# disanda/Deep-GAN-Encoders

Measured on AMD Instinct MI355X. Metric: encoder-train images/sec (E_align_s2 step, StyleGAN2 FFHQ-1024), higher is better.
Workload: dtype bf16; 1 GPU; E_align_s2 two-phase step, StyleGAN2-1024 G (train mode) + BE(startf=16, L=9) + LPIPS-VGG16 (seeded stand-in weights), batch 8/GPU; global_batch=8, img_size=1024, parallelism=dp1

## Files before the change

### deep-gan-encoders_amd/_lib.py

```python
import ctypes as C
import os

_HERE = os.path.dirname(os.path.abspath(__file__))
LIB_PATH = os.environ.get("DGE_LIB_PATH", os.path.join(_HERE, "libdge_hip.so"))


class DgeError(RuntimeError):
    pass


class ConvDesc(C.Structure):
    _fields_ = [
        ("x", C.c_void_p), ("w_packed", C.c_void_p), ("y", C.c_void_p), ("addend", C.c_void_p), ("dot_src", C.c_void_p),
        ("in_scale", C.c_void_p), ("in_shift", C.c_void_p), ("out_scale", C.c_void_p),
        ("bias", C.c_void_p), ("noise", C.c_void_p), ("noise_w", C.c_void_p), ("stats", C.c_void_p),
        ("B", C.c_int), ("H", C.c_int), ("W", C.c_int), ("Cin", C.c_int), ("Cout", C.c_int),
        ("ksize", C.c_int), ("up", C.c_int), ("in_s2d", C.c_int), ("noise_batch", C.c_int), ("noise_w_per_channel", C.c_int),
        ("act", C.c_int), ("bias_scale", C.c_float), ("gain", C.c_float), ("add_scale", C.c_float),
        ("dtype", C.c_int), ("in_up2", C.c_int), ("in_relu", C.c_int), ("stats_slots", C.c_int), ("w_layout", C.c_int),
        ("prep", C.c_int), ("prep_gain", C.c_float), ("prep_noise", C.c_void_p), ("prep_ns", C.c_void_p), ("prep_noise_batch", C.c_int),
        ("prep_stats", C.c_void_p), ("mask_relu", C.c_int), ("in_t2d", C.c_int),
        ("rgb_w", C.c_void_p), ("rgb_style", C.c_void_p), ("rgb_bias", C.c_void_p), ("rgb_out", C.c_void_p), ("rgb_wscale", C.c_float),
        ("rgb_skip_y", C.c_int), ("pool_out", C.c_int), ("pool_mask", C.c_void_p),
        ("prefetch_w", C.c_void_p), ("prefetch_ntot", C.c_int), ("prefetch_cin", C.c_int), ("in_bwd_coef", C.c_void_p),
# ... 88 lines not shown
    "dge_heads_rows_fwd": [_P, _I, _P, _P, C.c_long, C.c_long, _I, _I, _I, _P],
    "dge_heads_rows_bwd": [_P, _I, _I, _P, C.c_long, C.c_long, _I, _P, _P, _P, _P, _I, _I, _P],
    "dge_dense_wgrad": [_P, _I, _P, _I, _P, _P, _I, _I, _I, _I, _P],
    "dge_lpips_prep": [_P, _P, _I, _I, _I, _P, _P, _I, _P],
    "dge_lpips_prep_bwd": [_P, _P, _I, _I, _I, _P, _F, _I, _I, _P],
    "dge_maxpool2": [_P, _P, _I, _I, _I, _I, _I, _P],
    "dge_maxpool2_bwd": [_P, _P, _P, _P, _I, _I, _I, _I, _I, _P],
    "dge_lpips_head": [_P, _P, _P, _P, _I, _I, _I, _F, _I, _P],
    "dge_mean": [_P, _P, _I, _P],
    "dge_blur_noise_act": [_P, _P, _P, _P, _P, _P, _I, _I, _I, _I, _I, _I, _I, _I, _P],
    "dge_affine_compose": [_P, _P, _P, _P, _P, _I, _I, _P],
    "dge_lerp_layers": [_P, _P, _I, _P, _P, _I, _I, _I, _P],
    "dge_linear_rows": [_P, _I, _P, _P, _P, _P, _P, _P, _I, _I, _I, _F, _F, _F, _P],
    "dge_demod_rows": [_P, _P, _P, _P, _P, _P, _P, _P, _I, _I, _F, _P],
    "dge_fromrgb_dgrad": [_P, _P, _P, _P, _I, _I, _I, _I, _P],
    "dge_nearest_up2": [_P, _P, _I, _I, _I, _I, _F, _I, _P],
    "dge_sg1_in_bwd_coef": [_P, _P, _P, _P, _P, _P, _I, _I, _I, _P],
    "dge_dot_stats": [_P, _P, _P, _I, _I, _I, _I, _P],
    "dge_nearest_up2_bwd": [_P, _P, _P, _P, _I, _I, _I, _I, _I, _P],
    "dge_pixelnorm_nhwc": [_P, _P, C.c_long, _I, _F, _I, _P],
    "dge_pixelnorm_nhwc_bwd": [_P, _P, _P, C.c_long, _I, _F, _I, _P],
    "dge_affine_relu_bwd": [_P, _P, _P, _P, _P, _P, _I, _I, _I, _I, _P],
    "dge_slice_up_bwd": [_P, _P, _I, _I, _I, _I, _I, _I, _I, _P],
    "dge_softmax_rows": [_P, C.c_long, _I, _I, _P],
    "dge_softmax_rows_bwd": [_P, _P, C.c_long, _I, _I, _P],
    "dge_rgb_tanh_bwd": [_P, _P, _P, _I, _I, _I, _I, _P],
    "dge_sn_group": [_P, _I, _I, _I, _P, _F, _I, _P],
    "dge_sn_entry_size": [],
    "dge_cbn_sn_wgrad_entry_size": [],
    "dge_cbn_sn_wgrad_group": [_P, _I, C.c_longlong, _I, _P, _I, _I, _P, _P],
    "dge_upconv_supported": [_I, _I, _I],
    "dge_pack_upconv_weight": [_P, _P, _I, _I, _F, _I, _P],
    "dge_upconv_fir": [_P, _P, _P, _P, _P, _P, _I, _P, _I, _P, _F, _F, _I, _I, _I, _I, _I, _I, _I, _P],
    "dge_cbn_affine": [_P, _P, _I, _P, _P, _F, _P, _P, _I, _I, _P],
    "dge_slice_up": [_P, _P, _I, _I, _I, _I, _I, _I, _I, _P],
    "dge_attention": [_P, _P, _P, _P, _I, _I, _I, _I, _I, _I, _P],
    "dge_rgb_tanh": [_P, _P, _I, _I, _I, _I, _P],
    "dge_guided_relu_bwd": [_P, _P, _P, C.c_long, _I, _I, _P],
    "dge_maxpool2_relu_bwd": [_P, _P, _P, _I, _I, _I, _I, _I, _I, _P],
    "dge_maxpool2_bwd_relu": [_P, _P, _P, _P, _I, _I, _I, _I, _I, _P],
    "dge_adaptive_pool7": [_P, _P, _I, _I, _I, _I, _I, _P],
    "dge_adaptive_pool7_bwd": [_P, _P, _I, _I, _I, _I, _I, _P],
    "dge_class_target": [_P, _P, _P, _P, _I, _I, _P],
    "dge_gather_row": [_P, _P, _P, _I, _I, _F, _P],
    "dge_class_target_rows": [_P, _P, _P, _P, _I, _I, _P],
    "dge_gather_rows": [_P, _P, _P, _I, _I, _P],
    "dge_campp_map": [_P, _P, _P, _P, _P, _I, _I, _I, _I, _I, _P],
    "dge_cam_resize": [_P, _P, _P, _I, _I, _I, _I, _I, _P],
    "dge_mask2cam_blocks": [_I],
    "dge_mask2cam": [_P, _P, _P, _P, _P, _P, _P, _I, _I, _P],
    "dge_mask2cam_rows": [_P, _P, _P, _P, _P, _P, _I, _I, _P],
    "dge_randn": [_P, _I, _P, _P, _P, _P, C.c_ulonglong, _P, _P],
    "dge_version": [],
    "dge_env_reload": [],
    "dge_blend_pool_mask": [_P, _P, _P, _P, _P, _I, _I, _I, _I, _F, _F, _I, _P],
    "dge_act_bwd_mask": [_P, _P, _P, _P, _P, _I, _I, _I, _I, _I, _F, _F, _I, _P],
    "dge_loss_reduce3": [_P, _P, _P, _I, _I, _I, _I, _P, _I, _P],
    "dge_crop_pool_multi": [_P, _P, _P, _P, _I, _I, _I, _I, _P],
    "dge_space_loss_bwd3": [_P, _P, _P, _P, _P, _I, _I, _I, _P, _P, _P, _P, _I, _P],
    "dge_space_loss_bwd_split": [_P, _P, _P, _P, _P, _I, _I, _I, _P, _P, _P, _P, _I, _P],
    "dge_in_bwd_fromrgb": [_P, _P, _P, _I, _P, _P, _P, _P, _I, _P, _P, _P, _I, _I, _I, _I, _I, _F, _I, _P],
    "dge_in_bwd_fromrgb_img": [_P, _P, _P, _I, _P, _P, _P, _P, _I, _P, _P, _P, _P, _P, _I, _I, _I, _I, _I, _F, _I, _P],
    "dge_affine_bwd_fromrgb_img": [_P, _P, _P, _P, _P, _P, _P, _P, _I, _I, _I, _I, _I, _F, _I, _P],
    "dge_in_bwd_fused": [_P, _P, _P, _I, _P, _P, _P, _P, _I, _P, _P, _P, _P, _I, _I, _I, _I, _I, _F, _I, _I, _P],
    "dge_sum_slots_planar_multi": [C.POINTER(SumPlanarEntry), _I, _P],
    "dge_heads_fwd": [_P, _I, _P, _P, _I, _I, _I, _P],
# ... 56 lines not shown
```

### deep-gan-encoders_amd/autograd_s2.py

```python
import torch

from . import ops, s2_conv
from .stylegan2_generator import _dt
from .weight_cache import version


def _style_tables(mod, B, dt):
    nl = mod.num_layers
    groups = [(getattr(mod, f"layer{i}"), i) for i in range(nl - 1)] + [(getattr(mod, f"output{k}"), 2 * k + 1) for k in range(nl // 2)]
    key = (B, str(dt)) + tuple(version(p) for L, _ in groups for p in (L.style.weight, L.style.bias, L.weight))
    cache = mod.__dict__.setdefault("_style_tab", {})
    hit = cache.get(key[:2])
    if hit is not None and hit[0] == key:
        return hit[1]
    dev = groups[0][0].weight.device
    K = mod.w_space_dim
    Wc = torch.cat([L.style.weight.detach() for L, _ in groups]).contiguous()
    bc = torch.cat([L.style.bias.detach() for L, _ in groups]).contiguous()
    xoff, ybase, ybs, s_off = [], [], [], []
    off = 0
    for L, row in groups:
        C = L.in_c
        s_off.append(B * off)
        xoff += [row * K] * C
# ... 91 lines not shown
        g_x, g_srgb, P = ops.torgb_bwd_prep(g_img, layers[top]["y"], Ot.weight.detach().reshape(3, -1), saved["rgb"][top // 2]["s"], Ot.wscale,
                                            layers[top]["noise"], Lt.noise_strength.detach().reshape(1), Lt.gain)
    else:
        g_x, g_srgb = ops.torgb_bwd(g_img, layers[top]["y"], Ot.weight.detach().reshape(3, -1), saved["rgb"][top // 2]["s"], Ot.wscale)
    blocks = [] if fused else None
    if fused:
        blocks.append(dict(gs=g_srgb, wstyle=Ot.style.weight.detach(), row=top + 1))
    else:
        ops.linear_t(g_srgb, Ot.style.weight.detach(), g_wp[:, top + 1], scale=Ot.style.wscale, accumulate=True)
    if top // 2 > 0:
        g_img = ops.up2_bwd(g_img)
    for i in range(top, -1, -1):
        L = getattr(mod, f"layer{i}")
        rec = layers[i]
        if P is not None:
            g_y, d_in = g_x, rec["d"]
        else:
            R = ops.zeros((B, L.out_c, 3), dev)
            g_y, d_in = ops.modconv_bwd_prep(g_x, rec["y"], rec["d"], rec["noise"], L.gain, R), None
        x_in = saved["const"] if i == 0 else layers[i - 1]["y"]
        addend = None
        if i >= 1 and (i - 1) % 2 == 0:
            kp = (i - 1) // 2
            Op = getattr(mod, f"output{kp}")
            addend, g_srgb = ops.torgb_bwd(g_img, x_in, Op.weight.detach().reshape(3, -1), saved["rgb"][kp]["s"], Op.wscale)
            if fused:
                blocks.append(dict(gs=g_srgb, wstyle=Op.style.weight.detach(), row=i))
            else:
                ops.linear_t(g_srgb, Op.style.weight.detach(), g_wp[:, i], scale=Op.style.wscale, accumulate=True)
            if kp > 0:
                g_img = ops.up2_bwd(g_img)
        st = ops.SlotStats(B, L.in_c, dev) if fused else ops.zeros((B, L.in_c, 2), dev)
        prep, P_next = None, None
        if fused and i >= 1 and s2_conv.dgrad_takes_prep(L):
            Lp = getattr(mod, f"layer{i - 1}")
            P_next = ops.SlotStats(B, L.in_c, dev)
            prep = dict(gain=Lp.gain, noise=layers[i - 1]["noise"], ns=Lp.noise_strength.detach().reshape(1), stats=P_next)
        g_xprev = s2_conv.dgrad(L, g_y, d_in, dt, fused, prep=prep, out_scale=rec["s"], addend=addend, stats=st, dot_src=x_in)
        _, wsq = L._prepared(dt)
        if fused and P is not None:
            blocks.append(dict(P=P, st=st, d=rec["d"], s=rec["s"], bias=L.bias.detach(), wsq=wsq, bscale=L.bscale,
                               wstyle=L.style.weight.detach(), row=i))
            g_x, P = g_xprev, P_next
            continue
        if fused:
            st_t = ops.zeros((B, L.in_c, 2), dev)
            ops.check(ops.lib().dge_sum_slots(ops._p(st.buf), ops._p(st_t), st.nslot, st_t.numel(), 0, ops._stream()), "dge_sum_slots")
            st = st_t
        if P is not None:
            t = ops.demod_bwd_prep(P, rec["d"], L.bias.detach(), L.bscale)
        else:
            t = ops.demod_bwd(R, rec["d"], L.bias.detach(), L.noise_strength.detach().reshape(1), L.bscale)
        gs_view = st.view(B, -1)
        ops.linear_t(t, wsq, gs_view, mul=rec["s"], accumulate=True, incy=2, ldy=2 * L.in_c)
        ops.linear_t(gs_view, L.style.weight.detach(), g_wp[:, i], scale=L.style.wscale, accumulate=True, incx=2,
                     ldx=2 * L.in_c, O=L.in_c)
        g_x, P = g_xprev, P_next
    if blocks:
        ops.s2_style_grads(blocks, g_wp, getattr(mod, "layer0").style.wscale)
    return g_wp


class SynthesisFunction(torch.autograd.Function):
    @staticmethod
    def forward(ctx, mod, wp, randomize_noise):
        need = ctx.needs_input_grad[1]
        results, saved = synthesis_run(mod, wp.detach(), randomize_noise, save=need)
# ... 32 lines not shown
```

### deep-gan-encoders_amd/ops.py

```python
import ctypes as C
import math

import torch

from ._lib import lib, check, ConvDesc, ConvPPDesc, DgeError, last_kernel

F32, BF16 = 0, 1
ACT_NONE, ACT_LRELU, ACT_RELU, LIN_RSQRT = 0, 1, 2, 3
PACK_FWD, PACK_UPFOLD, PACK_DGRAD, PACK_UPFOLD_DGRAD, PACK_SG1_UP, PACK_SG1_UP_DGRAD, PACK_UPT2D_DGRAD = 0, 1, 2, 3, 4, 5, 6
PACK_FRAG = 0x100
import os as _os
import weakref as _weakref
KERNEL_LOG = None
PROFILE = None


class _ZeroArena:

    def __init__(self):
        self.buf, self.off, self.high, self.active = None, 0, 0, False


_ARENA = _ZeroArena()

# ... 1146 lines not shown

def maxpool2_bwd(gy, x, addend=None, relu=False):
    B, H, W, Cc = x.shape
    gx = torch.empty_like(x)
    fn = lib().dge_maxpool2_bwd_relu if relu else lib().dge_maxpool2_bwd
    check(fn(_p(gy), _p(x), _p(addend), _p(gx), B, H, W, Cc, dtype_of(x), _stream()), "dge_maxpool2_bwd")
    return gx


def upconv_supported(cin, cout, dtype):
    return bool(lib().dge_upconv_supported(int(cin), int(cout), int(dtype)))


def pack_upconv_weight(w, dtype=BF16, scale=1.0):
    cout, cin = w.shape[0], w.shape[1]
    out = torch.empty((9, cout, cin), dtype=tdtype(dtype), device=w.device)
    check(lib().dge_pack_upconv_weight(_f32(w.detach().contiguous()), _p(out), cout, cin, float(scale), dtype, _stream()),
          "dge_pack_upconv_weight")
    return out


def upconv_fir(x, w_packed, cout, in_scale=None, out_scale=None, bias=None, bias_scale=1.0, noise=None, noise_w=None,
               act=ACT_NONE, gain=1.0):
    B, H, W, Cin = x.shape
    y = torch.empty((B, 2 * H, 2 * W, cout), dtype=x.dtype, device=x.device)
    nbs = 0 if (noise is None or noise.shape[0] == 1) else 4 * H * W
    nws = 0 if (noise_w is None or noise_w.numel() == 1) else 1
    _launch(lib().dge_upconv_fir, (_p(x), _p(w_packed), _p(y), _f32(in_scale), _f32(out_scale), _f32(noise), nbs, _f32(noise_w), nws,
                                   _f32(bias), float(bias_scale), float(gain), int(act), B, H, W, Cin, cout, dtype_of(x), _stream()),
            "dge_upconv_fir", 9.0 * Cin * cout * H * W * B, (B, H, W, Cin, cout, 3, "upfir", False), (x, y, w_packed))
    return y


TRACK_ARM_AT, TRACK_ARM_AFTER = 0, 1


def latent_pnorm(w, p=2, out=None, out_l2=None):
    if out is None:
        out = torch.empty((), dtype=torch.float32, device=w.device)
    check(lib().dge_latent_pnorm_fwd(_f32(w.contiguous()), _p(out), _f32(out_l2), w.numel(), int(p), _stream()), "dge_latent_pnorm_fwd")
    return out


def latent_l2(w, out=None):
    if out is None:
        out = torch.empty((), dtype=torch.float32, device=w.device)
    check(lib().dge_latent_pnorm_fwd(_f32(w.contiguous()), None, _p(out), w.numel(), 2, _stream()), "dge_latent_pnorm_fwd")
    return out


def latent_pnorm_bwd(w, norm, g, p=2, beta=1.0, gout=None):
    check(lib().dge_latent_pnorm_bwd(_f32(w.contiguous()), _f32(norm), _f32(gout), _f32(g), w.numel(), int(p), float(beta), _stream()),
          "dge_latent_pnorm_bwd")
    return g


def wplus_lerp(w, avg, psi, out=None):
    B, L, D = w.shape
    if out is None:
        out = torch.empty((B, L, D), dtype=torch.float32, device=w.device)
    stride = D if avg.numel() == L * D else 0
    check(lib().dge_wplus_lerp(_f32(w.contiguous()), _f32(avg.contiguous()), stride, float(psi), _p(out), B, L, D, _stream()),
          "dge_wplus_lerp")
    return out


# ... 59 lines not shown
```

### deep-gan-encoders_amd/s2_conv.py

```python
import os

from . import ops
from .weight_cache import lookup, store

PP_GEN = not os.environ.get("DGE_NO_PP_GEN")
UP_PP = os.environ.get("DGE_UP_PP", "1") != "0"
UP_FOLDED = os.environ.get("DGE_UP_FOLDED") == "1"
T2D = not os.environ.get("DGE_NO_T2D")
PP_DG = not os.environ.get("DGE_NO_PP_DG")


def prepared(L, dtype):
    c = lookup(L._cache, ("w", dtype), L.weight)
    if c is None:
        mode = ops.PACK_UPFOLD if L.up else ops.PACK_FWD
        hin = L.res // 2 if L.up else L.res
        packed = ops.pack_conv_weight(L.weight, ops.pack_mode_for(L.weight, mode, hin, hin, dtype), dtype, L.wscale) \
            if L.ksize == 3 else None
        wsq = ops.weight_sumsq(L.weight, L.wscale) if L.demodulate else None
        c = store(L._cache, ("w", dtype), L.weight, (packed, wsq))
    return c


def _prepared_up(L, dtype):
    if not L.up or L.res < 32 or UP_FOLDED or not ops.upconv_supported(L.in_c, L.out_c, dtype):
        return None
    c = lookup(L._cache, ("wu", dtype), L.weight)
    return c if c is not None else store(L._cache, ("wu", dtype), L.weight, ops.pack_upconv_weight(L.weight, dtype, L.wscale))


def forward(L, x, s, d, noise, dt, rgb=None):
    nw = L.noise_strength.detach().reshape(1) if noise is not None else None
    B, H, W, _ = x.shape
    wu = _prepared_up(L, dt)
    if wu is not None:
        assert rgb is None
        if (UP_PP and s is not None and d is not None and (noise is None or nw.numel() == 1)
                and ops.up_pp_supported(B, H, W, L.in_c, L.out_c, dt)):
            wimg = ops.pack_up_pp(wu, L.out_c, L.in_c, in_scale=s, out_scale=d, gain=L.gain)
            return ops.up_pp(x, wimg, L.out_c, bias=L.bias, bias_scale=L.bscale, noise=noise, noise_w=nw, act=L.act, gain=L.gain)
        return ops.upconv_fir(x, wu, L.out_c, in_scale=s, out_scale=d, bias=L.bias, bias_scale=L.bscale, noise=noise, noise_w=nw, act=L.act, gain=L.gain)
    if (rgb is None and not L.up and d is not None and s is not None and L.ksize == 3 and PP_GEN
# ... 4 lines not shown
    return ops.conv2d(x, packed, L.out_c, 3, up=L.up, in_scale=s, out_scale=d, bias=L.bias, bias_scale=L.bscale, noise=noise, noise_w=nw, act=L.act, gain=L.gain, rgb=rgb)


def _up_phase_form(L):
    return L.up and 32 <= L.res // 2 <= 128 and L.in_c >= 64 and L.in_c % 32 == 0 and L.out_c % 8 == 0 and T2D


def _dgrad_weight(L, dtype):
    hg = L.res // 2 if L.up else L.res
    if _up_phase_form(L):
        mode = ops.PACK_UPT2D_DGRAD
    else:
        mode = ops.pack_mode_for(L.weight, ops.PACK_UPFOLD_DGRAD if L.up else ops.PACK_DGRAD, hg, hg, dtype)
    c = lookup(L._cache, ("dg", dtype, mode), L.weight)
    return c if c is not None else store(L._cache, ("dg", dtype, mode), L.weight, ops.pack_conv_weight(L.weight, mode, dtype, L.wscale))


def _pp_dgrad(L, B, hg, dtype):
    K = 4 * L.out_c if L.up else L.out_c
    return PP_DG and (not L.up or L.out_c % 32 == 0) and ops.conv_pp_supported(B, hg, hg, K, L.in_c, dtype)


def _dgrad_weight_pp(L, d, t2d=False):
    if not L.up:
        return ops.pack_conv_pp(L.weight, L.wscale, in_scale=d, dgrad=True)
    name = "dgpp_t2d" if t2d else "dgpp"
    c = lookup(L._cache, name, L.weight)
    if c is None:
        rows = ops.pack_conv_weight(L.weight, ops.PACK_UPT2D_DGRAD if t2d else ops.PACK_UPFOLD_DGRAD, ops.F32, L.wscale)
        c = store(L._cache, name, L.weight, ops.pack_conv_pp_rows(rows, L.in_c, t2d=True) if t2d else rows)
    return c if t2d else ops.pack_conv_pp_rows(c, L.in_c, in_scale=d, in_period=L.out_c)


def dgrad_takes_prep(L):
    return _up_phase_form(L) or not (L.up and L.in_c < 128)


def dgrad(L, g_y, d_in, dt, fused, prep=None, **epilogue):
    B, hg = g_y.shape[0], (L.res // 2 if L.up else L.res)
    t2d = _up_phase_form(L)
    if fused and d_in is not None and not t2d and _pp_dgrad(L, B, hg, dt):
        return ops.conv_pp(g_y, _dgrad_weight_pp(L, d_in), L.in_c, dgrad=True, in_s2d=L.up, add_scale=1.0, prep=prep, **epilogue)
    if t2d and fused and prep is not None and _pp_dgrad(L, B, hg, dt):
        return ops.conv_pp(ops.fir_t2d(g_y, d_in), _dgrad_weight_pp(L, None, t2d=True), L.in_c, dgrad=True, in_t2d=True, add_scale=1.0, prep=prep, **epilogue)
    if t2d:
        return ops.conv2d(ops.fir_t2d(g_y, d_in), _dgrad_weight(L, dt), L.in_c, 3, in_t2d=True, add_scale=1.0, prep=prep, **epilogue)
    return ops.conv2d(g_y, _dgrad_weight(L, dt), L.in_c, 3, in_s2d=L.up, in_scale=d_in, add_scale=1.0, prep=prep, **epilogue)
```

### include/dge_hip.h

```cpp
#ifndef DGE_HIP_H
#define DGE_HIP_H
#include <stddef.h>
#ifdef __cplusplus
extern "C" {
#endif

typedef struct ihipStream_t* dge_stream_t;

#define DGE_DTYPE_F32 0
#define DGE_DTYPE_BF16 1
#define DGE_ACT_LINEAR 0
#define DGE_ACT_LRELU02 1
#define DGE_ACT_RELU_ 2
#define DGE_LIN_RSQRT 3
#define DGE_PACK_FWD 0
#define DGE_PACK_UPFOLD 1
#define DGE_PACK_DGRAD 2
#define DGE_PACK_UPFOLD_DGRAD 3
#define DGE_PACK_SG1_UP 4
#define DGE_PACK_SG1_UP_DGRAD 5
#define DGE_PACK_UPT2D_DGRAD 6

const char* dge_last_error(void);
int dge_version(void);
// ... 212 lines not shown
int dge_maxpool2(const void* x, void* y, int B, int H, int W, int C, int dtype, dge_stream_t stream);
int dge_maxpool2_bwd(const void* gy, const void* x, const void* addend, void* gx, int B, int H, int W, int C, int dtype,
                     dge_stream_t stream);
int dge_lpips_head(const void* feat, const float* lin, float* val, void* g1, int B, int HW, int C, float gscale, int dtype,
                   dge_stream_t stream);
int dge_mean(const float* v, float* out, int n, dge_stream_t stream);

int dge_blur_noise_act(const void* x, const float* noise, const float* noise_w, const float* bias, void* y, float* stats,
                       int B, int H, int W, int C, int do_blur, int noise_batch, int act, int dtype, dge_stream_t stream);
int dge_affine_compose(const float* sc, const float* sh, const float* style, float* a, float* b, int B, int C, dge_stream_t stream);
int dge_lerp_layers(const float* w, const float* avg, int avg_stride, const float* coefs, float* out, int B, int L, int D,
                    dge_stream_t stream);

int dge_sg1_in_bwd_coef(const float* dots, const float* sc, const float* sh, const float* style, float* coef, float* gstyle,
                        int B, int C, int npix, dge_stream_t stream);
int dge_dot_stats(const void* g, const void* x, float* stats, int B, int HW, int C, int dtype, dge_stream_t stream);
int dge_nearest_up2_bwd(const void* ghi, const void* x, void* glow, float* stats, int B, int H, int W, int C, int dtype,
                        dge_stream_t stream);

int dge_sn_group(const void* entries, int n, int maxO, int maxK, float* sigma, float eps, int training, dge_stream_t stream);
int dge_sn_entry_size(void);
int dge_cbn_sn_wgrad_entry_size(void);
int dge_cbn_sn_wgrad_group(const void* entries, int n, long long rows, int maxC, const float* cond, int B, int K, float* rowdot, dge_stream_t stream);

int dge_randn(float* out, int nseg, const long long* start, const long long* count, const unsigned long long* goff,
              const unsigned int* subseq, unsigned long long seed, const unsigned long long* seed_dev, dge_stream_t stream);

int dge_upconv_supported(int Cin, int Cout, int dtype);
int dge_pack_upconv_weight(const float* w, void* out, int Cout, int Cin, float scale, int dtype, dge_stream_t stream);
int dge_upconv_fir(const void* x, const void* w_packed, void* y, const float* in_scale, const float* out_scale,
                   const float* noise, int noise_bstride, const float* noise_w, int noise_w_stride, const float* bias,
                   float bias_scale, float gain, int act, int B, int H, int W, int Cin, int Cout, int dtype, dge_stream_t stream);

int dge_up_pp_supported(int B, int H, int W, int Cin, int Cout, int dtype);
int dge_pack_up_pp(const void* w_units, void* out, int Cout, int Cin, const float* in_scale, const float* out_scale, float gain,
                   int nb, dge_stream_t stream);
int dge_up_pp(const void* x, const void* w_img, long long w_bstride, void* y, const float* noise, int noise_bstride,
              const float* noise_w, const float* bias, float bias_scale, float gain, int act, int B, int H, int W, int Cin, int Cout,
              dge_stream_t stream);

typedef struct dge_conv_pp_desc {
    const void* x;
    const void* w_pp;
    void* y;
    long long w_bstride;
    const float* out_scale;
    const float* bias;
    const float* noise;
    const float* noise_w;
    int B, H, W, Cin, Cout;
    int noise_batch;
    int noise_w_per_channel;
    int act;
    float bias_scale, gain;
    int dgrad, in_s2d, stats_slots, prep, prep_noise_batch, mask_relu;
    int in_t2d;
    float add_scale, prep_gain;
    const void* dot_src;
    const void* addend;
    float* stats;
    float* prep_stats;
    const float* prep_noise;
    const float* prep_ns;
} dge_conv_pp_desc;
int dge_conv_pp_supported(int B, int H, int W, int Cin, int Cout, int dtype);
int dge_pack_conv_pp(const float* w_oihw, void* out, int N, int K, float wscale, const float* in_scale, const float* out_scale,
// ... 67 lines not shown
```

Baseline: 374.9 images/sec.

## Add streaming fused upsample-conv dgrad kernel for 64<-32 channel layers

Adds a dedicated HIP kernel for the backward data gradient of the upsampling 3x3 modulated conv at the highest-resolution 64->32 channel StyleGAN2 layer. It streams gradient rows through LDS with direct-to-LDS buffer loads, applies the transposed FIR blur in registers, runs MFMA, and fuses the epilogue: out_scale, addend, dot-product stats, and the previous layer's prep (lrelu gain, noise, stats). This removes the separate FIR-transpose pass and the generic conv path, plus their intermediate memory traffic. It only handles one channel configuration, is disabled in deterministic mode, and lets that layer take the fused prep path.

```diff
diff --git a/deep-gan-encoders_amd/_lib.py b/deep-gan-encoders_amd/_lib.py
--- a/deep-gan-encoders_amd/_lib.py
+++ b/deep-gan-encoders_amd/_lib.py
@@ -144,6 +144,8 @@
     "dge_upconv_supported": [_I, _I, _I],
     "dge_pack_upconv_weight": [_P, _P, _I, _I, _F, _I, _P],
     "dge_upconv_fir": [_P, _P, _P, _P, _P, _P, _I, _P, _I, _P, _F, _F, _I, _I, _I, _I, _I, _I, _I, _P],
+    "dge_up_dgrad_stream_supported": [_I, _I, _I, _I, _I, _I],
+    "dge_up_dgrad_stream": [_P, _P, _P, _P, _P, _P, _P, _P, _I, _I, _F, _P, _I, _P, _P, _I, _I, _I, _I, _I, _I, _P],
     "dge_cbn_affine": [_P, _P, _I, _P, _P, _F, _P, _P, _I, _I, _P],
     "dge_slice_up": [_P, _P, _I, _I, _I, _I, _I, _I, _I, _P],
     "dge_attention": [_P, _P, _P, _P, _I, _I, _I, _I, _I, _I, _P],
diff --git a/deep-gan-encoders_amd/autograd_s2.py b/deep-gan-encoders_amd/autograd_s2.py
--- a/deep-gan-encoders_amd/autograd_s2.py
+++ b/deep-gan-encoders_amd/autograd_s2.py
@@ -147,7 +147,7 @@
                 g_img = ops.up2_bwd(g_img)
         st = ops.SlotStats(B, L.in_c, dev) if fused else ops.zeros((B, L.in_c, 2), dev)
         prep, P_next = None, None
-        if fused and i >= 1 and s2_conv.dgrad_takes_prep(L):
+        if fused and i >= 1 and s2_conv.dgrad_takes_prep(L, B, dt):
             Lp = getattr(mod, f"layer{i - 1}")
             P_next = ops.SlotStats(B, L.in_c, dev)
             prep = dict(gain=Lp.gain, noise=layers[i - 1]["noise"], ns=Lp.noise_strength.detach().reshape(1), stats=P_next)
diff --git a/deep-gan-encoders_amd/csrc/upconv_stream_bwd.hip b/deep-gan-encoders_amd/csrc/upconv_stream_bwd.hip
--- /dev/null
+++ b/deep-gan-encoders_amd/csrc/upconv_stream_bwd.hip
@@ -0,0 +1,382 @@
+#include <type_traits>
+#include <stdlib.h>
+#include "common.h"
+#include "../../include/dge_hip.h"
+
+namespace {
+
+typedef __attribute__((ext_vector_type(4))) unsigned rsrc_t;
+typedef __attribute__((ext_vector_type(2))) float f2_t;
+
+__device__ __forceinline__ unsigned rfl(unsigned v) { return __builtin_amdgcn_readfirstlane(v); }
+__device__ __forceinline__ unsigned lds_off(const void* p) {
+    return (unsigned)(size_t)(const __attribute__((address_space(3))) unsigned char*)p;
+}
+__device__ __forceinline__ rsrc_t make_rsrc(unsigned long long base, unsigned bytes) {
+    rsrc_t r;
+    r[0] = rfl((unsigned)base); r[1] = rfl((unsigned)(base >> 32) & 0xffffu); r[2] = rfl(bytes); r[3] = 0x00020000u;
+    return r;
+}
+
+struct UpbParams {
+    const void* gz; const void* w; void* y; const void* addend; const void* dot_src;
+    const float* d_in; const float* out_scale;
+    float* stats; float* prep_stats; int stats_slots;
+    const float* prep_noise; const float* prep_ns; int prep_noise_bstride; float prep_gain;
+    int B, H, W;
+    int nstrips, nseg, seg_rows, njobs, jobs_per_xcd;
+    int dbg;
+};
+
+constexpr int CIN = 64, COUT = 32;
+constexpr int ZRB = 34 * 128;
+constexpr int NS = 3, D = 2;
+constexpr int ZPAIR = 2 * ZRB;
+constexpr int Z_OFF = 0;
+constexpr int T_OFF = (NS * ZPAIR + 255) / 256 * 256;
+constexpr int T_ODD = 34 * 64;
+constexpr int TRB = T_ODD + 32 * 64, NT = 4;
+constexpr int D_OFF = T_OFF + NT * TRB;
+constexpr int DROWB = 2048, DRING = NS * DROWB;
+constexpr int A_OFF = D_OFF + 2 * DRING;
+constexpr int N_OFF = A_OFF + 2 * DRING;
+constexpr int NRING = NS * 256;
+constexpr int DUMMY_OFF = (N_OFF + 2 * NRING + 255) / 256 * 256;
+constexpr int LDS_BYTES = DUMMY_OFF + 1024;
+constexpr int LPR = 6 + 2 + 2 + 1;
+static_assert((D - 1) * LPR < 64, "vmcnt range");
+
+__device__ __forceinline__ int swz8(int px) { return (px >> 1) & 7; }
+__device__ __forceinline__ int swz4(int px) { return (px >> 2) & 3; }
+
+#define UPB_P(off) "buffer_load_dwordx4 %1, %3, 0 offen offset:" #off " lds\n\t"
+#define UPB_M0 "s_mov_b32 m0, %2\n\ts_nop 0\n\t"
+__device__ __forceinline__ void dma_row(int wave, unsigned voff, unsigned voff_b, unsigned voff_c, rsrc_t rs, rsrc_t rs_null,
+                                        unsigned m0v, unsigned m0_dummy) {
+    unsigned long long keep;
+    if (wave == 0)
+        asm volatile(UPB_M0 UPB_P(0) UPB_P(2048)
+                     "s_mov_b32 m0, %5\n\ts_mov_b64 %0, exec\n\ts_mov_b64 exec, 0xffff\n\tbuffer_load_dwordx4 %4, %3, 0 offen lds\n\ts_mov_b64 exec, %0"
+                     : "=&s"(keep) : "v"(voff), "s"(m0v), "s"(rs), "v"(voff_c), "s"(m0v + 4096u) : "memory");
+    else
+        asm volatile(UPB_M0 UPB_P(1024) UPB_P(3072) "s_mov_b32 m0, %5\n\ts_nop 0\n\tbuffer_load_dwordx4 %1, %4, 0 offen lds"
+                     : "=&s"(keep) : "v"(voff_b), "s"(m0v), "s"(rs), "s"(rs_null), "s"(m0_dummy) : "memory");
+}
+__device__ __forceinline__ void dma_half(unsigned voff, unsigned voff1, rsrc_t rs, unsigned m0v) {
+    asm volatile("s_mov_b32 m0, %1\n\ts_nop 0\n\tbuffer_load_dwordx4 %0, %2, 0 offen lds\n\t"
+                 "buffer_load_dwordx4 %3, %2, 0 offen offset:1024 lds" : : "v"(voff), "s"(m0v), "s"(rs), "v"(voff1) : "memory");
+}
+__device__ __forceinline__ void dma_f32(unsigned voff, rsrc_t rs, unsigned m0v) {
+    asm volatile("s_mov_b32 m0, %1\n\ts_nop 0\n\tbuffer_load_dword %0, %2, 0 offen lds" : : "v"(voff), "s"(m0v), "s"(rs) : "memory");
+}
+
+__device__ __forceinline__ int chan_of_row(int m) {
+    const int j = m >> 3, k = (m >> 2) & 1, i = m & 3;
+    return 16 * (j >> 1) + 8 * k + 4 * (j & 1) + i;
+}
+__device__ __forceinline__ int chan_of_reg(int kh, int r) { return (r < 8 ? 8 * kh + r : 16 + 8 * kh + (r - 8)); }
+
+template <bool PREP>
+__global__ __launch_bounds__(128, 1) void upconv_stream_bwd_kernel(UpbParams p) {
+    extern __shared__ __attribute__((aligned(1024))) unsigned char lds[];
+    const int lane = threadIdx.x & 63;
+    const int wave = (int)rfl(threadIdx.x >> 6);
+    const unsigned lds0 = lds_off(lds);
+    const int n31 = lane & 31, kh = lane >> 5;
+
+    int job = (blockIdx.x & 7) * p.jobs_per_xcd + (blockIdx.x >> 3);
+    if ((int)(blockIdx.x >> 3) >= p.jobs_per_xcd || job >= p.njobs) return;
+    const int strip = job % p.nstrips; job /= p.nstrips;
+    const int seg = job % p.nseg;
+    const int b = job / p.nseg;
+    const int r0 = seg * p.seg_rows;
+    const int r1 = min(r0 + p.seg_rows, p.H);
+    const int nsteps = r1 - r0 + 2;
+    const int x0 = 32 * strip;
+    const int FH = 2 * p.H;
+
+    const unsigned zrow_bytes = (unsigned)(2 * p.W) * (COUT * 2);
+    const unsigned yrow_bytes = (unsigned)p.W * (CIN * 2);
+    const unsigned long long Zb = (unsigned long long)p.gz + (unsigned long long)b * FH * zrow_bytes;
+    const unsigned long long DOTb = (unsigned long long)p.dot_src + (unsigned long long)b * p.H * yrow_bytes;
+    const unsigned long long ADDb = p.addend ? (unsigned long long)p.addend + (unsigned long long)b * p.H * yrow_bytes : Zb;
+    const bool has_nz = PREP && p.prep_noise != nullptr;
+    const unsigned long long NZb = has_nz ? (unsigned long long)(p.prep_noise + (size_t)b * p.prep_noise_bstride) : Zb;
+    const unsigned nzrow_bytes = (unsigned)p.W * 4;
+
+    unsigned voff, voff_b, voff_c;
+    {
+        const int px = lane >> 3, cs = lane & 7;
+        const int gx = x0 - 1 + px;
+        voff = (unsigned)(gx * 128 + ((cs ^ swz8(px)) << 4));
+        voff_b = (unsigned)(gx * 128 + ((cs ^ swz8(px + 8)) << 4));
+        voff_c = voff + 4096;
+    }
+    unsigned dvoff, dvoff1;
+    {
+        const int px = lane >> 2, cs = lane & 3;
+        dvoff = (unsigned)((x0 + px) * 128 + wave * 64 + ((cs ^ swz4(px)) << 4));
+        dvoff1 = dvoff + 2048u - 1024u;
+    }
+    const unsigned nvoff = lane < 32 ? (unsigned)((x0 + lane) * 4) : 0x80000000u;
+    const rsrc_t rs_null = make_rsrc(Zb, 0);
+
+    auto issue = [&](int tt, int slot) {
+        const int gy = 2 * (r0 - 1 + tt);
+        const bool live = tt < nsteps;
+        const bool zv = live && gy >= 0 && gy < FH;
+        const unsigned long long zp = Zb + (unsigned long long)(zv ? gy : 0) * zrow_bytes;
+        const unsigned m0z = lds0 + Z_OFF + (unsigned)slot * ZPAIR;
+        dma_row(wave, voff, voff_b, voff_c, make_rsrc(zp, zv ? zrow_bytes : 0u), rs_null, m0z, lds0 + DUMMY_OFF);
+        dma_row(wave, voff, voff_b, voff_c, make_rsrc(zp + zrow_bytes, zv ? zrow_bytes : 0u), rs_null, m0z + ZRB, lds0 + DUMMY_OFF);
+        const bool ov = live && tt >= 2;
+        const unsigned long long ro = (unsigned long long)(ov ? r0 - 2 + tt : 0);
+        dma_half(dvoff, dvoff1, make_rsrc(DOTb + ro * yrow_bytes, ov ? yrow_bytes : 0u), lds0 + D_OFF + (unsigned)(wave * DRING + slot * DROWB));
+        dma_half(dvoff, dvoff1, make_rsrc(ADDb + ro * yrow_bytes, (ov && p.addend) ? yrow_bytes : 0u), lds0 + A_OFF + (unsigned)(wave * DRING + slot * DROWB));
+        dma_f32(nvoff, make_rsrc(NZb + ro * nzrow_bytes, (ov && has_nz) ? nzrow_bytes : 0u), lds0 + N_OFF + (unsigned)(wave * NRING + slot * 256));
+    };
+    asm volatile("s_waitcnt vmcnt(0)" ::: "memory");
+    for (int h = 0; h < D; h++) issue(h, h);
+
+    uint4 wf[9][2];
+    {
+        const bf16_t* __restrict__ Wp = (const bf16_t*)p.w;
+        const int ci = wave * 32 + chan_of_row(n31);
+#pragma unroll
+        for (int tap = 0; tap < 9; tap++)
+#pragma unroll
+            for (int ks = 0; ks < 2; ks++) wf[tap][ks] = *(const uint4*)(Wp + ((size_t)(tap * CIN + ci) * COUT + ks * 16 + kh * 8));
+    }
+    float oscv[16];
+#pragma unroll
+    for (int r = 0; r < 16; r++) oscv[r] = p.out_scale ? p.out_scale[b * CIN + wave * 32 + chan_of_reg(kh, r)] : 1.f;
+    const float pg_pos = p.prep_gain, pg_neg = 0.2f * p.prep_gain, pz_pos = 1.f / p.prep_gain, pz_neg = 1.f / (0.2f * p.prep_gain);
+    const float pns = (has_nz && p.prep_ns) ? p.prep_ns[0] : 0.f;
+
+    typedef unsigned u32x4_t __attribute__((ext_vector_type(4)));
+    typedef const __attribute__((address_space(3))) u32x4_t* lds_u4p;
+    typedef __attribute__((address_space(3))) u32x4_t* lds_u4wp;
+    typedef const __attribute__((address_space(3))) float* lds_fp;
+    auto lds_u4 = [&](unsigned a) { const u32x4_t t = *(lds_u4p)(size_t)a; return make_uint4(t[0], t[1], t[2], t[3]); };
+    auto lds_st4 = [&](unsigned a, unsigned v0, unsigned v1, unsigned v2, unsigned v3) { u32x4_t t; t[0] = v0; t[1] = v1; t[2] = v2; t[3] = v3; *(lds_u4wp)(size_t)a = t; };
+
+    const int fc = lane & 3, fj = lane >> 2;
+    unsigned zoff[6];
+#pragma unroll
+    for (int k = 0; k < 6; k++) {
+        const int sp = 16 * wave + fj + (k >> 1);
+        zoff[k] = lds0 + Z_OFF + (unsigned)(sp * 128 + ((((k & 1) * 4 + fc) ^ swz8(sp)) << 4));
+    }
+    const int tj = 16 * wave + fj;
+    const unsigned toff_e = lds0 + T_OFF + (unsigned)(tj * 64 + ((fc ^ swz4(tj)) << 4));
+    const unsigned toff_o = toff_e + T_ODD;
+    const unsigned toff_x = lds0 + T_OFF + (unsigned)((tj + 1) * 64 + ((fc ^ swz4(tj + 1)) << 4));
+    const bool wr_x = tj == 31;
+    f2_t dsc[4];
+#pragma unroll
+    for (int i = 0; i < 4; i++) dsc[i] = p.d_in ? f2_t{p.d_in[b * COUT + 8 * fc + 2 * i], p.d_in[b * COUT + 8 * fc + 2 * i + 1]} : f2_t{1.f, 1.f};
+    f2_t hist[3][3][4];
+#pragma unroll
+    for (int r = 0; r < 3; r++)
+#pragma unroll
+        for (int c = 0; c < 3; c++)
+#pragma unroll
+            for (int i = 0; i < 4; i++) hist[r][c][i] = f2_t{0.f, 0.f};
+
+    unsigned boff[3][2];
+#pragma unroll
+    for (int kx = 0; kx < 3; kx++)
+#pragma unroll
+        for (int ks = 0; ks < 2; ks++) {
+            const int jj = n31 + (kx >> 1);
+            boff[kx][ks] = lds0 + T_OFF + (unsigned)((kx & 1) * T_ODD + jj * 64 + (((2 * ks + kh) ^ swz4(jj)) << 4));
+        }
+    unsigned eoff[2];
+#pragma unroll
+    for (int q = 0; q < 2; q++) eoff[q] = (unsigned)(wave * DRING + n31 * 64 + (((2 * q + kh) ^ swz4(n31)) << 4));
+    const unsigned nzoff = lds0 + N_OFF + (unsigned)(wave * NRING + n31 * 4);
+
+    const bool pv = x0 + n31 < p.W;
+    const bool stv = pv && !(p.dbg & 1);
+    unsigned char* __restrict__ Yb = (unsigned char*)p.y + (size_t)b * p.H * yrow_bytes + (size_t)(x0 + n31) * (CIN * 2) + wave * 64 + kh * 16;
+    float s0[16], s1[16], s2[PREP ? 16 : 1];
+#pragma unroll
+    for (int r = 0; r < 16; r++) { s0[r] = 0.f; s1[r] = 0.f; if (PREP) s2[r] = 0.f; }
+    f32x16_t zero16;
+#pragma unroll
+    for (int r = 0; r < 16; r++) zero16[r] = 0.f;
+
+    int slot = 0, slot_pf = D % NS;
+    for (int t = 0; t < nsteps; t++) {
+        asm volatile("s_waitcnt vmcnt(%0)" :: "i"((D - 1) * LPR) : "memory");
+        __builtin_amdgcn_s_barrier();
+        issue(t + D, slot_pf);
+
+        if (!(p.dbg & 8)) {
+            f2_t hn[2][3][4];
+#pragma unroll
+            for (int r = 0; r < 2; r++) {
+                f2_t g[6][4];
+#pragma unroll
+                for (int k = 0; k < 6; k++) {
+                    const uint4 v = lds_u4(zoff[k] + (unsigned)(slot * ZPAIR + r * ZRB));
+                    const unsigned w4[4] = {v.x, v.y, v.z, v.w};
+#pragma unroll
+                    for (int i = 0; i < 4; i++) g[k][i] = f2_t{__uint_as_float(w4[i] << 16), __uint_as_float(w4[i] & 0xffff0000u)};
+                }
+#pragma unroll
+                for (int c = 0; c < 3; c++)
+#pragma unroll
+                    for (int i = 0; i < 4; i++) hn[r][c][i] = (g[c][i] + g[c + 3][i]) * 0.25f + (g[c + 1][i] + g[c + 2][i]) * 0.75f;
+            }
+            const unsigned ta = (unsigned)(((2 * t + 1) & (NT - 1)) * TRB), tb = (unsigned)(((2 * t + 2) & (NT - 1)) * TRB);
+#pragma unroll
+            for (int c = 0; c < 3; c++) {
+                unsigned oa[4], ob[4];
+#pragma unroll
+                for (int i = 0; i < 4; i++) {
+                    const f2_t va = ((hist[0][c][i] + hn[0][c][i]) * 0.25f + (hist[1][c][i] + hist[2][c][i]) * 0.75f) * dsc[i];
+                    const f2_t vb = ((hist[1][c][i] + hn[1][c][i]) * 0.25f + (hist[2][c][i] + hn[0][c][i]) * 0.75f) * dsc[i];
+                    oa[i] = pack2bf(va[0], va[1]); ob[i] = pack2bf(vb[0], vb[1]);
+                    hist[0][c][i] = hist[2][c][i]; hist[1][c][i] = hn[0][c][i]; hist[2][c][i] = hn[1][c][i];
+                }
+                const unsigned o = c == 0 ? toff_e : (c == 1 ? toff_o : toff_x);
+                if (c < 2 || wr_x) { lds_st4(o + ta, oa[0], oa[1], oa[2], oa[3]); lds_st4(o + tb, ob[0], ob[1], ob[2], ob[3]); }
+            }
+        }
+        asm volatile("s_waitcnt lgkmcnt(0)" ::: "memory");
+        __builtin_amdgcn_s_barrier();
+
+        if (t >= 2) {
+            constexpr int NQ = 18, PF = 6;
+            unsigned rowb[3];
+#pragma unroll
+            for (int ky = 0; ky < 3; ky++) rowb[ky] = (unsigned)(((2 * t + ky) & (NT - 1)) * TRB);
+            f32x16_t acc = zero16;
+            if (!(p.dbg & 2)) {
+                uint4 bq[PF];
+                StaticFor<PF>::run([&](auto qc) { constexpr int q = decltype(qc)::value; bq[q] = lds_u4(boff[(q >> 1) % 3][q & 1] + rowb[(q >> 1) / 3]); });
+                StaticFor<NQ>::run([&](auto qc) {
+                    constexpr int q = decltype(qc)::value;
+                    constexpr int tap = q >> 1, ks = q & 1;
+                    const bf16x8_t bf = *(const bf16x8_t*)&bq[q % PF];
+                    acc = __builtin_amdgcn_mfma_f32_32x32x16_bf16(*(const bf16x8_t*)&wf[tap][ks], bf, acc, 0, 0, 0);
+                    if constexpr (q + PF < NQ) { constexpr int q2 = q + PF; bq[q % PF] = lds_u4(boff[(q2 >> 1) % 3][q2 & 1] + rowb[(q2 >> 1) / 3]); }
+                });
+            }
+            const unsigned so = (unsigned)(slot * DROWB);
+            uint4 dd[2], aa[2];
+#pragma unroll
+            for (int q = 0; q < 2; q++) { dd[q] = lds_u4(lds0 + D_OFF + eoff[q] + so); aa[q] = lds_u4(lds0 + A_OFF + eoff[q] + so); }
+            float nzs = 0.f;
+            if (PREP) nzs = pns * *(lds_fp)(size_t)(nzoff + (unsigned)(slot * 256));
+            float v[16];
+#pragma unroll
+            for (int q = 0; q < 2; q++) {
+                float dv[8], av[8];
+                unpack16(dd[q], dv, (bf16_t*)nullptr);
+                unpack16(aa[q], av, (bf16_t*)nullptr);
+#pragma unroll
+                for (int e = 0; e < 8; e++) {
+                    const int r = 8 * q + e;
+                    const float a = acc[r];
+                    s0[r] = fmaf(a, dv[e], s0[r]);
+                    const float g = fmaf(a, oscv[r], av[e]);
+                    if (PREP) {
+                        const bool pos = dv[e] > 0.f;
+                        const float gz = g * (pos ? pg_pos : pg_neg);
+                        const float zt = dv[e] * (pos ? pz_pos : pz_neg) - nzs;
+                        s2[PREP ? r : 0] = fmaf(gz, zt, s2[PREP ? r : 0]); s1[r] += gz;
+                        v[r] = gz;
+                    } else {
+                        s1[r] += a;
+                        v[r] = g;
+                    }
+                }
+            }
+            if (stv) {
+                unsigned char* dst = Yb + (size_t)(r0 - 2 + t) * yrow_bytes;
+                *(uint4*)dst = make_uint4(pack2bf(v[0], v[1]), pack2bf(v[2], v[3]), pack2bf(v[4], v[5]), pack2bf(v[6], v[7]));
+                *(uint4*)(dst + 32) = make_uint4(pack2bf(v[8], v[9]), pack2bf(v[10], v[11]), pack2bf(v[12], v[13]), pack2bf(v[14], v[15]));
+            }
+        }
+        slot = slot + 1 == NS ? 0 : slot + 1;
+        slot_pf = slot_pf + 1 == NS ? 0 : slot_pf + 1;
+    }
+    asm volatile("s_waitcnt vmcnt(0)" ::: "memory");
+
+    if (p.stats) {
+        float* __restrict__ ST = p.stats + ((size_t)(blockIdx.x % p.stats_slots) * p.B + b) * CIN * 2;
+        float* __restrict__ PST = (PREP && p.prep_stats) ? p.prep_stats + ((size_t)(blockIdx.x % p.stats_slots) * p.B + b) * CIN * 2 : nullptr;
+        float va = 0.f, vc = 0.f, vt = 0.f;
+#pragma unroll
+        for (int r = 0; r < 16; r++) {
+            float a = pv ? s0[r] : 0.f, c = pv ? s1[r] : 0.f, t2 = (PREP && pv) ? s2[PREP ? r : 0] : 0.f;
+#pragma unroll
+            for (int m = 1; m < 32; m <<= 1) {
+                a += __shfl_xor(a, m, 64); c += __shfl_xor(c, m, 64);
+                if (PREP) t2 += __shfl_xor(t2, m, 64);
+            }
+            if (n31 == r) { va = a; vc = c; vt = t2; }
+        }
+        if (n31 < 16) {
+            const int ch = wave * 32 + chan_of_reg(kh, n31);
+            atomicAdd(ST + ch * 2, va);
+            if (PREP) { if (PST) { atomicAdd(PST + ch * 2, vt); atomicAdd(PST + ch * 2 + 1, vc); } }
+            else atomicAdd(ST + ch * 2 + 1, vc);
+        }
+    }
+}
+
+template <bool PREP>
+int launch(UpbParams& p, hipStream_t s) {
+    auto kern = upconv_stream_bwd_kernel<PREP>;
+    static int caps[16] = {0};
+    int dev = 0;
+    (void)hipGetDevice(&dev);
+    int& cap = caps[dev >= 0 && dev < 16 ? dev : 0];
+    if (!cap) {
+        (void)hipFuncSetAttribute((const void*)kern, hipFuncAttributeMaxDynamicSharedMemorySize, LDS_BYTES);
+        int occ = 0, ncu = 256;
+        (void)hipDeviceGetAttribute(&ncu, hipDeviceAttributeMultiprocessorCount, dev);
+        if (hipOccupancyMaxActiveBlocksPerMultiprocessor(&occ, (const void*)kern, 128, LDS_BYTES) != hipSuccess || occ < 1) occ = 1;
+        cap = occ * ncu;
+    }
+    p.nstrips = (p.W + 31) / 32;
+    int nseg = cap / (p.B * p.nstrips);
+    int maxseg = p.H / 16; if (maxseg < 1) maxseg = 1;
+    if (nseg > maxseg) nseg = maxseg;
+    if (nseg < 1) nseg = 1;
+    p.seg_rows = (p.H + nseg - 1) / nseg;
+    p.nseg = (p.H + p.seg_rows - 1) / p.seg_rows;
+    p.njobs = p.B * p.nstrips * p.nseg;
+    p.jobs_per_xcd = (p.njobs + 7) / 8;
+    dge_note_kernel(PREP ? "upconv_stream_bwd<bf16,%d,%d>+prep" : "upconv_stream_bwd<bf16,%d,%d>", CIN, COUT);
+    hipLaunchKernelGGL(kern, dim3((unsigned)(p.jobs_per_xcd * 8)), dim3(128), LDS_BYTES, s, p);
+    DGE_LAUNCH_CHECK("upconv_stream_bwd");
+    return 0;
+}
+
+}
+
+extern "C" int dge_up_dgrad_stream_supported(int B, int H, int W, int Cin, int Cout, int dtype) {
+    if (dtype != DGE_BF16 || Cin != CIN || Cout != COUT || B < 1 || H < 1 || W < 1) return 0;
+    if ((long)W * 128 >= (1L << 31) || (long)B * H * W * 128 >= (1L << 40)) return 0;
+    return 1;
+}
+
+extern "C" int dge_up_dgrad_stream(const void* g_z, const void* w_packed, void* y, const float* d_in, const float* out_scale,
+                                   const void* addend, const void* dot_src, float* stats, int stats_slots, int prep, float prep_gain,
+                                   const float* prep_noise, int prep_noise_bstride, const float* prep_ns, float* prep_stats,
+                                   int B, int H, int W, int Cin, int Cout, int dtype, hipStream_t s) {
+    DGE_CHECK(dge_up_dgrad_stream_supported(B, H, W, Cin, Cout, dtype), "up_dgrad_stream: bf16, %d -> %d channels only (got %d -> %d)", CIN, COUT, Cin, Cout);
+    DGE_CHECK(dot_src && stats && stats_slots >= 1, "up_dgrad_stream: needs dot_src and stats");
+    DGE_CHECK(!prep || (prep_stats && prep_gain > 0.f), "up_dgrad_stream: prep needs its stats and a positive gain");
+    UpbParams p;
+    p.gz = g_z; p.w = w_packed; p.y = y; p.addend = addend; p.dot_src = dot_src; p.d_in = d_in; p.out_scale = out_scale;
+    p.stats = stats; p.prep_stats = prep ? prep_stats : nullptr; p.stats_slots = stats_slots;
+    p.prep_noise = prep ? prep_noise : nullptr; p.prep_ns = prep_ns; p.prep_noise_bstride = prep_noise_bstride; p.prep_gain = prep ? prep_gain : 1.f;
+    p.B = B; p.H = H; p.W = W;
+    p.dbg = dge_env().up_dbg;
+    return prep ? launch<true>(p, s) : launch<false>(p, s);
+}
diff --git a/deep-gan-encoders_amd/ops.py b/deep-gan-encoders_amd/ops.py
--- a/deep-gan-encoders_amd/ops.py
+++ b/deep-gan-encoders_amd/ops.py
@@ -1202,6 +1202,47 @@
     return y
 
 
+def up_dgrad_stream_supported(B, Hin, Win, cin, cout, dtype):
+    return (not is_deterministic()) and bool(lib().dge_up_dgrad_stream_supported(int(B), int(Hin), int(Win), int(cin), int(cout), int(dtype)))
+
+
+def pack_up_dgrad_stream(w, dtype=BF16, scale=1.0):
+    if dtype != BF16:
+        raise DgeError("pack_up_dgrad_stream: bf16 only")
+    cout, cin = w.shape[0], w.shape[1]
+    return (w.detach().float() * float(scale)).flip(2, 3).permute(2, 3, 1, 0).reshape(9, cin, cout).to(torch.bfloat16).contiguous()
+
+
+def up_dgrad_stream(g_z, w_packed, d_in, out_scale, addend, stats, dot_src, prep=None):
+    B, FH, FW, cout = g_z.shape
+    H, W = FH // 2, FW // 2
+    _, cin, _ = w_packed.shape
+    dt = dtype_of(g_z)
+    if dot_src is None or stats is None:
+        raise DgeError("up_dgrad_stream: needs stats and dot_src")
+    if not up_dgrad_stream_supported(B, H, W, cin, cout, dt):
+        raise DgeError(f"up_dgrad_stream: unsupported launch {cin} <- {cout} channels, dtype {dt}")
+    out = torch.empty((B, H, W, cin), dtype=g_z.dtype, device=g_z.device)
+    nslot = _stats_slots(B, H, W, 32)
+    lazy = isinstance(stats, SlotStats)
+    partial = stats.alloc(nslot) if lazy else (zeros((nslot,) + tuple(stats.shape), g_z.device) if nslot > 1 else stats)
+    pn = pns = pst = None
+    pgain, pbs = 1.0, 0
+    if prep is not None:
+        pn = prep.get("noise")
+        pns = prep.get("ns") if pn is not None else None
+        pbs = 0 if (pn is None or pn.shape[0] == 1) else H * W
+        pgain, pst = float(prep["gain"]), prep["stats"].alloc(nslot)
+    _launch(lib().dge_up_dgrad_stream,
+            (_p(g_z), _p(w_packed), _p(out), _f32(d_in), _f32(out_scale), _p(addend), _p(dot_src), _f32(partial), nslot,
+             0 if prep is None else 1, pgain, _f32(pn), pbs, _f32(pns), _f32(pst), B, H, W, cin, cout, dt, _stream()),
+            "dge_up_dgrad_stream", 9.0 * cin * cout * H * W * B, (B, H, W, 4 * cout, cin, 3, False, True),
+            (g_z, out, addend, dot_src, w_packed))
+    if not lazy and partial is not stats:
+        check(lib().dge_sum_slots(_p(partial), _p(stats), nslot, stats.numel(), 1, _stream()), "dge_sum_slots")
+    return out
+
+
 TRACK_ARM_AT, TRACK_ARM_AFTER = 0, 1
 
 
diff --git a/deep-gan-encoders_amd/s2_conv.py b/deep-gan-encoders_amd/s2_conv.py
--- a/deep-gan-encoders_amd/s2_conv.py
+++ b/deep-gan-encoders_amd/s2_conv.py
@@ -8,6 +8,7 @@
 UP_FOLDED = os.environ.get("DGE_UP_FOLDED") == "1"
 T2D = not os.environ.get("DGE_NO_T2D")
 PP_DG = not os.environ.get("DGE_NO_PP_DG")
+UP_DG_STREAM = not os.environ.get("DGE_NO_UP_DG_STREAM")
 
 
 def prepared(L, dtype):
@@ -78,12 +79,27 @@
     return c if t2d else ops.pack_conv_pp_rows(c, L.in_c, in_scale=d, in_period=L.out_c)
 
 
-def dgrad_takes_prep(L):
+def _up_stream_dgrad(L, B, dtype, fused):
+    return UP_DG_STREAM and fused and L.up and L.ksize == 3 and ops.up_dgrad_stream_supported(B, L.res // 2, L.res // 2, L.in_c, L.out_c, dtype)
+
+
+def _dgrad_weight_stream(L, dtype):
+    c = lookup(L._cache, ("dgs", dtype), L.weight)
+    return c if c is not None else store(L._cache, ("dgs", dtype), L.weight, ops.pack_up_dgrad_stream(L.weight, dtype, L.wscale))
+
+
+def dgrad_takes_prep(L, B=None, dtype=None):
+    if B is not None and L.up and _up_stream_dgrad(L, B, dtype, not ops.is_deterministic()):
+        return True
     return _up_phase_form(L) or not (L.up and L.in_c < 128)
 
 
 def dgrad(L, g_y, d_in, dt, fused, prep=None, **epilogue):
     B, hg = g_y.shape[0], (L.res // 2 if L.up else L.res)
+    if L.up and _up_stream_dgrad(L, B, dt, fused) and epilogue.get("dot_src") is not None and epilogue.get("stats") is not None \
+            and set(epilogue) <= {"out_scale", "addend", "stats", "dot_src"}:
+        return ops.up_dgrad_stream(g_y, _dgrad_weight_stream(L, dt), d_in, epilogue.get("out_scale"), epilogue.get("addend"),
+                                   epilogue.get("stats"), epilogue["dot_src"], prep=prep)
     t2d = _up_phase_form(L)
     if fused and d_in is not None and not t2d and _pp_dgrad(L, B, hg, dt):
         return ops.conv_pp(g_y, _dgrad_weight_pp(L, d_in), L.in_c, dgrad=True, in_s2d=L.up, add_scale=1.0, prep=prep, **epilogue)
diff --git a/include/dge_hip.h b/include/dge_hip.h
--- a/include/dge_hip.h
+++ b/include/dge_hip.h
@@ -268,6 +268,12 @@
                    const float* noise, int noise_bstride, const float* noise_w, int noise_w_stride, const float* bias,
                    float bias_scale, float gain, int act, int B, int H, int W, int Cin, int Cout, int dtype, dge_stream_t stream);
 
+int dge_up_dgrad_stream_supported(int B, int H, int W, int Cin, int Cout, int dtype);
+int dge_up_dgrad_stream(const void* g_z, const void* w_packed, void* y, const float* d_in, const float* out_scale,
+                        const void* addend, const void* dot_src, float* stats, int stats_slots, int prep, float prep_gain,
+                        const float* prep_noise, int prep_noise_bstride, const float* prep_ns, float* prep_stats,
+                        int B, int H, int W, int Cin, int Cout, int dtype, dge_stream_t stream);
+
 int dge_up_pp_supported(int B, int H, int W, int Cin, int Cout, int dtype);
 int dge_pack_up_pp(const void* w_units, void* out, int Cout, int Cin, const float* in_scale, const float* out_scale, float gain,
                    int nb, dge_stream_t stream);
```

After: 379.1 images/sec (median of 6 runs). +1.1%, better.
